# chrismile/Correrender

Hardware: AMD Instinct MI355X
Metric: Mvoxel-corr/s (higher is better)
Workload: dtype f32; 1 GPU; pearson correlation field, 256x256x256 grid x 64 ensemble members (synthetic box ensemble), one moving reference point per step; members=64, measure=pearson, resident=members and result in HBM

## Files before the change

### correrender_amd/csrc/api.cpp

```cpp
#include "../../include/corrfield.h"

#include <hip/hip_runtime.h>

#include <cstdarg>
#include <cstdlib>
#include <cstdio>
#include <cmath>
#include <cstring>
#include <functional>
#include <immintrin.h>
#include <sys/mman.h>

#include <algorithm>
#include <atomic>
#include <chrono>
#include <limits>
#include <memory>
#include <string>
#include <thread>
#include <vector>

#include "crf_context.h"
#include "crf_host_copy.h"
#include "crf_internal.h"
// ... 312 lines not shown
    if (int(current.ptrs.size()) != c->cs)
        return fail(c, CRF_ERR_STATE, "no member volumes uploaded or bound");
    return CRF_OK;
}

crf::Event take_event(crf_context* c) {
    crf::Event e;
    if (!c->ev_free.empty()) {
        e = std::move(c->ev_free.back());
        c->ev_free.pop_back();
    } else {
        (void)e.create();
    }
    return e;
}

hipStream_t stream_of(crf_context* c, void* stream) { return stream ? static_cast<hipStream_t>(stream) : c->stream; }

int launch_status(crf_context* c, hipError_t e) {
    if (e == hipSuccess) return CRF_OK;
    return fail(c, CRF_ERR_DEVICE, fmt("kernel launch failed: %s", hipGetErrorString(e)));
}

struct TimedLaunch {
    crf_context* c;
    crf::Event e0, e1;
    crf::LaunchInfo info;
    explicit TimedLaunch(crf_context* ctx, bool timed = true) : c(ctx) {
        if (c->profiling && timed) {
            e0 = take_event(c);
            e1 = take_event(c);
        }
    }
    int finish(hipError_t e) {
        c->last_kernel = info.kernel_name ? info.kernel_name : "";
        if (e0 && e1) c->ev_pending.emplace_back(std::move(e0), std::move(e1));
        return launch_status(c, e);
    }
};

int check_params(crf_context* c, const crf_params* p, int member_limit, const char* who = nullptr) {
    if (!p) return fail(c, CRF_ERR_ARGUMENT, "null argument");
    if (p->measure < CRF_PEARSON || p->measure > CRF_KMI_CC)
        return fail(c, CRF_ERR_ARGUMENT, fmt("unknown measure %d", p->measure));
    for (int v : p->reserved)
        if (v != 0) return fail(c, CRF_ERR_ARGUMENT, "crf_params.reserved must be zero");
    if (member_limit > 0 && c->cs > member_limit)
        return fail(c, CRF_ERR_UNSUPPORTED,
                    who ? fmt("%s at most %d members", who, member_limit)
                        : fmt("measure %d supports at most %d members (got %d)", p->measure, member_limit, c->cs));
    if ((p->measure == CRF_MI_BINNED || p->measure == CRF_BINNED_MI_CC) && (p->num_bins < 1 || p->num_bins > 255))
        return fail(c, CRF_ERR_ARGUMENT, fmt("num_bins %d outside [1,255]", p->num_bins));
    if ((p->measure == CRF_MI_KRASKOV || p->measure == CRF_KMI_CC) && p->k < 1)
        return fail(c, CRF_ERR_ARGUMENT, fmt("k=%d must be at least 1", p->k));
    return CRF_OK;
}

int check_slots(crf_context* c, int first, int count, bool one = false) {
    if (count >= 0 && first >= 0 && first + count <= CRF_PREPARED_SLOTS) return CRF_OK;
    return fail(c, CRF_ERR_ARGUMENT,
                one ? fmt("slot %d outside [0,%d)", first, CRF_PREPARED_SLOTS)
                    : fmt("slots [%d, %d) outside [0, %d)", first, first + count, CRF_PREPARED_SLOTS));
}

size_t launch_voxels(const crf_context* c) { return c->pipeline_voxels ? c->pipeline_voxels : c->view.num_voxels; }

int ensure_workspace(crf_context* c, size_t need) {
    for (int set = 0; set < c->pipeline_sets; set++) {
        crf_scratch& sc = c->grid.scratch[set];
// ... 363 lines not shown
                break;
            }
            e = crf::launch_mi_kraskov(c->view.members, c->cs, c->view.num_voxels, ref, ka, c->grid.tables.get(), prep, out, s,
                                       e0, e1, info);
            break;
        }
    }
    const int rc = launch.finish(e);
    if (e == hipErrorNotSupported)
        return fail(c, CRF_ERR_UNSUPPORTED, fmt("measure %d is not implemented by this build", p->measure));
    return rc;
}

int compute_impl(crf_context* c, const crf_params* p, const void* device_reference_values, void* device_out,
                 void* stream, unsigned phase, int slot, const crf::RefOverride* ov = nullptr) {
    if (!c || !c->windowed || !p || (p->flags & CRF_FLAG_SYMMETRIC))
        return compute_impl_one(c, p, device_reference_values, device_out, stream, phase, slot, ov);
    if (int r = ensure_wide(c, stream_of(c, stream))) return r;
    if (phase & 1u)
        if (int r = compute_impl_one(c, p, device_reference_values, nullptr, stream, 1u, slot, ov)) return r;
    if (!(phase & 2u)) return CRF_OK;
    if (!device_out) return fail(c, CRF_ERR_ARGUMENT, "null argument");
    return for_each_window(c, static_cast<float*>(device_out), [&](float* o) {
        return compute_impl_one(c, p, nullptr, o, stream, 2u, slot, nullptr);
    });
}

int apply_abs(crf_context* c, const crf_params* p, void* device_out, void* stream) {
    if (p->flags & CRF_FLAG_ABSOLUTE_VALUE)
        CRF_HIP(c, crf::launch_abs(static_cast<float*>(device_out), c->view.num_voxels, stream_of(c, stream)));
    return CRF_OK;
}

int ensure_host_ranges(crf_context* c, bool native) {
    crf_grid_state& g = c->grid;
    if (g.host_chunks > 0 && g.chunk_native == native) return CRF_OK;
    g.host_chunks = 0;
    const size_t n = c->alloc_voxels;
    const std::vector<size_t> first = crf::host_range_partition(n, env_int_or("CRF_HOST_CHUNKS", 0),
                                                                crf::parse_shares(getenv("CRF_HOST_SHARES")), kMaxHostChunks);
    const int ranges = int(first.size()) - 1;
    std::vector<const void*> table(size_t(ranges) * size_t(c->cs));
    const crf_member_set& set = native ? g.narrow : g.members;
    const size_t element = crf::member_format_bytes(set.format);
    for (int j = 0; j < ranges; j++)
        for (int m = 0; m < c->cs; m++)
            table[size_t(j) * size_t(c->cs) + size_t(m)] =
                static_cast<const char*>(set.ptrs[size_t(m)]) + first[size_t(j)] * element;
    CRF_HIP(c, g.chunk_tables.reserve(table.size()));
    CRF_HIP(c, hipMemcpy(g.chunk_tables.get(), table.data(), table.size() * sizeof(void*), hipMemcpyHostToDevice));
    CRF_HIP(c, c->copy_stream.create());
    for (int j = 0; j < ranges; j++) CRF_HIP(c, c->chunk_done[j].create(hipEventDisableTiming));
    for (int j = 0; j < ranges; j++) CRF_HIP(c, c->chunk_copied[j].create(hipEventDisableTiming));
    CRF_HIP(c, c->prep_done.create(hipEventDisableTiming));
    for (int j = 0; j <= ranges; j++) g.chunk_first[j] = first[size_t(j)];
    g.host_chunks = ranges;
    g.chunk_native = native;
    return CRF_OK;
}

template <class Launch>
int run_windowed(crf_context* c, void* device_out, void* stream, bool native, Launch&& launch) {
    if (int r = bind_device(c)) return r;
    hipStream_t s = stream_of(c, stream);
    if (!native)
        if (int r = ensure_wide(c, s)) return r;
// ... 410 lines not shown
                       void* stream) {
    if (p && p->prepared_slot != 0) {
        if (p->prepared_slot < 0 || p->prepared_slot > CRF_PREPARED_SLOTS)
            return fail(c, CRF_ERR_ARGUMENT, fmt("prepared_slot %d outside [0,%d]", p->prepared_slot, CRF_PREPARED_SLOTS));
        if (c && !c->prep_slots) return fail(c, CRF_ERR_STATE, "prepared_slot given but crf_prepare_device was never called");
        if (int r = compute_impl(c, p, nullptr, device_out, stream, 2u, p->prepared_slot - 1)) return r;
    } else {
        if (int r = compute_impl(c, p, device_reference_values, device_out, stream, 3u, -1)) return r;
    }
    return apply_abs(c, p, device_out, stream);
}

int crf_prepare_device(crf_context* c, const crf_params* p, const void* device_reference_values, int slot, void* stream) {
    return crf::prepare_device_ex(c, p, device_reference_values, slot, stream, nullptr);
}

int crf_prepare_rows_device(crf_context* c, const crf_params* p, const void* device_rows, int first_slot, int count,
                            void* stream) {
    if (!c || !p || !device_rows) return fail(c, CRF_ERR_ARGUMENT, "null argument");
    if (int r = check_slots(c, first_slot, count)) return r;
    crf_params local = *p;
    local.reference_values = nullptr;
    local.prepared_slot = 0;
    const float* rows = static_cast<const float*>(device_rows);
    for (int i = 0; i < count; i++)
        if (int r = crf_prepare_device(c, &local, rows + size_t(i) * size_t(c->cs), first_slot + i, stream)) return r;
    return CRF_OK;
}

int crf_compute_prepared_device(crf_context* c, const crf_params* p, int first_slot, int count, void* const* device_outs,
                                void* stream) {
    if (!c || !p || !device_outs) return fail(c, CRF_ERR_ARGUMENT, "null argument");
    if (int r = check_slots(c, first_slot, count)) return r;
    crf_params local = *p;
    for (int i = 0; i < count; i++) {
        local.prepared_slot = first_slot + i + 1;
        if (int r = crf_compute_device(c, &local, nullptr, device_outs[i], stream)) return r;
    }
    return CRF_OK;
}

int crf_compute(crf_context* c, const crf_params* p, float* host_out) {
    return crf::compute_to_host(c, p, nullptr, host_out, nullptr);
}

int crf_compute_requests_device(crf_context* c, const crf_params* p, const void* device_requests, size_t num_requests,
                                void* device_out, void* stream) {
    if (int r = check_ready(c)) return r;
    if (int r = check_params(c, p, crf::kMaxGenericMembers, "pair requests support")) return r;
    if (num_requests && (!device_requests || !device_out)) return fail(c, CRF_ERR_ARGUMENT, "null argument");
    if (c->windowed)
        return fail(c, CRF_ERR_UNSUPPORTED, "pair requests address voxels with 32-bit byte offsets: member volumes of 4 GiB or more are not supported in request mode");
    if (int r = bind_device(c)) return r;
    hipStream_t s = stream_of(c, stream);
    if (int r = ensure_wide(c, s)) return r;
    crf::TwoVectorJob job = two_vector_job(c, p);
    if (p->flags & CRF_FLAG_QUERY_FROM_SECONDARY) {
        if (!c->grid.has_secondary())
            return fail(c, CRF_ERR_STATE, "CRF_FLAG_QUERY_FROM_SECONDARY needs secondary members (crf_upload_secondary_members)");
        if (int r = ensure_secondary_wide(c, s)) return r;
        job.members_y = c->view.secondary;
    }
    job.requests = static_cast<const uint32_t*>(device_requests);
    job.num_items = num_requests;
    job.use_abs = (p->flags & CRF_FLAG_ABSOLUTE_VALUE) ? 1 : 0;
    job.out = static_cast<float*>(device_out);
// ... 292 lines not shown
    if (k < 1 || cs < 1) return std::numeric_limits<double>::quiet_NaN();
    return psi_int(cs) - psi_int(k);
}

size_t crf_tiled_element_count(int xs, int ys, int zs) {
    if (xs <= 0 || ys <= 0 || zs <= 0) return 0;
    return size_t((xs + 7) / 8) * size_t((ys + 7) / 8) * size_t((zs + 3) / 4) * 256;
}

int crf_tile_field_device(crf_context* c, const void* device_linear, void* device_tiled, void* stream) {
    if (!c) return CRF_ERR_ARGUMENT;
    if (c->cs <= 0) return fail(c, CRF_ERR_STATE, "crf_set_grid has not been called");
    if (c->windowed) return fail(c, CRF_ERR_UNSUPPORTED, "re-tiling a field of 4 GiB or more is not supported");
    if (!device_linear || !device_tiled) return fail(c, CRF_ERR_ARGUMENT, "null argument");
    if (int r = bind_device(c)) return r;
    hipStream_t s = stream_of(c, stream);
    hipError_t e = crf::launch_tile_field(static_cast<const float*>(device_linear), static_cast<float*>(device_tiled),
                                          c->xs, c->ys, c->zs, s);
    return launch_status(c, e);
}

int crf_set_profiling(crf_context* c, int enabled) {
    if (!c) return CRF_ERR_ARGUMENT;
    c->profiling = enabled != 0;
    return CRF_OK;
}

int crf_take_kernel_time(crf_context* c, double* out_ms_sum, int* out_launches) {
    if (!c || !out_ms_sum || !out_launches) return fail(c, CRF_ERR_ARGUMENT, "null argument");
    if (int r = bind_device(c)) return r;
    double sum = 0.0;
    int n = 0;
    for (auto& p : c->ev_pending) {
        CRF_HIP(c, hipEventSynchronize(p.second));
        float ms = 0.f;
        CRF_HIP(c, hipEventElapsedTime(&ms, p.first, p.second));
        sum += double(ms);
        n++;
        c->ev_free.push_back(std::move(p.first));
        c->ev_free.push_back(std::move(p.second));
    }
    c->ev_pending.clear();
    *out_ms_sum = sum;
    *out_launches = n;
    return CRF_OK;
}

const char* crf_last_kernel_name(const crf_context* c) { return c ? c->last_kernel.c_str() : ""; }

int crf_set_member_layout(crf_context* c, int mode) {
    if (!c) return CRF_ERR_ARGUMENT;
    if (mode != CRF_MEMBER_LAYOUT_AUTO && mode != CRF_MEMBER_LAYOUT_RAW && mode != CRF_MEMBER_LAYOUT_PACKED)
        return fail(c, CRF_ERR_ARGUMENT, fmt("unknown member layout %d", mode));
    if (mode == c->member_layout) return CRF_OK;
    if (int r = bind_device(c)) return r;
    CRF_HIP(c, hipDeviceSynchronize());
    drop_packed(c);
    c->member_layout = mode;
    return CRF_OK;
}

int crf_last_member_layout(const crf_context* c) { return c ? c->last_layout : CRF_MEMBER_LAYOUT_RAW; }

int crf_members_changed(crf_context* c) {
    if (!c) return CRF_ERR_ARGUMENT;
    if (int r = bind_device(c)) return r;
    CRF_HIP(c, hipDeviceSynchronize());
    primary_members_changed(c);
    secondary_members_changed(c);
    return CRF_OK;
}

int crf_synth_box_member(crf_context* c, void* device_out, int xs, int ys, int zs_local, int z_begin, int zs_global,
// ... 13 lines not shown
```

### correrender_amd/csrc/crf_context.h

```cpp
#pragma once
#include <hip/hip_runtime.h>

#include <atomic>
#include <memory>
#include <string>
#include <utility>
#include <vector>

#include "../../include/corrfield.h"
#include "crf_host_copy.h"
#include "crf_internal.h"
#include "crf_owned.h"
#include "crf_pool.h"
#include "crf_windows.h"

struct crf_scratch {
    crf::DeviceBuffer<uint32_t> todo;
    crf::DeviceBuffer<unsigned char> workspace;
};

struct crf_member_set {
    crf::DeviceBuffer<unsigned char> owned;
    std::vector<const void*> ptrs;
    crf::DeviceBuffer<const void*> table;
// ... 40 lines not shown
struct crf_launch_view {
    const float* const* members = nullptr;
    const float* const* secondary = nullptr;
    const void* const* narrow = nullptr;
    size_t num_voxels = 0;
    int max_vpt = 1;
    int scratch_set = 0;
    const void* const* secondary_narrow = nullptr;
};

struct crf_context {
    int device = -1;
    crf::Stream stream;
    std::string err;
    int xs = 0, ys = 0, zs = 0, cs = 0;
    size_t alloc_voxels = 0;
    bool windowed = false;
    size_t window_voxels = crf::kDefaultWindowVoxels;
    crf_grid_state grid;
    crf_launch_view view;
    int last_format = CRF_MEMBER_F32;
    int member_layout = CRF_MEMBER_LAYOUT_AUTO;
    int last_layout = CRF_MEMBER_LAYOUT_RAW;
    crf::DeviceBuffer<float> prep;
    crf::DeviceBuffer<float> prep_slots;
    crf::DeviceBuffer<uint32_t> minmax;
    crf::DeviceBuffer<uint32_t> pack_fallbacks;
    crf::DeviceBuffer<crf_request> requests;
    crf::DeviceBuffer<float> request_out;
    int pipeline_sets = 1;
    size_t pipeline_voxels = 0;
    bool profiling = false;
    std::vector<crf::Event> ev_free;
    std::vector<std::pair<crf::Event, crf::Event>> ev_pending;
    std::string last_kernel;
    std::atomic<int> chunk_ready[kMaxHostChunks] = {};
    crf::Stream stream2;
    crf::Stream copy_stream;
    crf::Event prep_done;
    crf::Event chunk_done[kMaxHostChunks];
    crf::Event chunk_copied[kMaxHostChunks];
    std::unique_ptr<crf::SpinPool> copy_pool;
    int copy_threads = 0;
    int copy_threads_cap = 0;
};


namespace crf {
inline hipError_t spin_on_event(hipEvent_t e) {
    const auto t0 = std::chrono::steady_clock::now();
    for (unsigned i = 1;; i++) {
        const hipError_t q = hipEventQuery(e);
        if (q != hipErrorNotReady) return q;
        if ((i & 1023u) == 0u && std::chrono::duration<double>(std::chrono::steady_clock::now() - t0).count() > 0.05)
            return hipEventSynchronize(e);
        _mm_pause();
    }
}
struct RefOverride {
    const float* const* table = nullptr;
    size_t voxel = 0;
};
int compute_to_host(crf_context* c, const crf_params* p, const void* device_reference_values, float* host_out,
                    const RefOverride* ref_override);
int compute_device_ex(crf_context* c, const crf_params* p, const void* device_reference_values, void* device_out,
                      void* stream, const RefOverride* ref_override);
int prepare_device_ex(crf_context* c, const crf_params* p, const void* device_reference_values, int slot, void* stream,
// ... 6 lines not shown
```

### correrender_amd/csrc/crf_internal.h

```cpp
#pragma once
#include <hip/hip_runtime.h>
#include <cstddef>
#include <cstdint>

#include "../../include/corrfield.h"
#include "symmetric_narrow_route.h"
#include "two_vector_route.h"

namespace crf {

constexpr int kMaxRegisterMembers = 384;
constexpr size_t kPrepBytes = 160 * 1024;
constexpr int kMaxGenericMembers = 2048;
constexpr size_t kBinnedSxOffset = kPrepBytes - 16;

struct RefSource {
    const float* values;
    size_t voxel;
    unsigned phase = 3;
    const float* const* table = nullptr;
    bool prepare() const { return (phase & 1u) != 0; }
    bool run() const { return (phase & 2u) != 0; }
};

// ... 39 lines not shown
}
__host__ __device__ inline uint32_t pack_lo16(uint32_t bits) { return bits & 0xFFFFu; }
__host__ __device__ inline uint32_t pack_byte(uint32_t bits) { return ((bits >> 24) & 0x80u) | ((bits >> 16) & 0x7Fu); }
__host__ __device__ inline uint32_t pack_code(uint32_t bits, uint32_t base) {
    const uint32_t e = (bits >> 23) & 0xFFu;
    return e == 0u ? 0u : e - base + 1u;
}
__host__ __device__ inline uint32_t perm_bytes(uint32_t hi, uint32_t lo, uint32_t sel) {
#if defined(__HIP_DEVICE_COMPILE__)
    return __builtin_amdgcn_perm(hi, lo, sel);
#else
    const uint64_t d = (uint64_t(hi) << 32) | lo;
    uint32_t r = 0;
    for (int i = 0; i < 4; i++) r |= uint32_t((d >> (8 * ((sel >> (8 * i)) & 7u))) & 0xFFu) << (8 * i);
    return r;
#endif
}
__host__ __device__ inline uint32_t unpack_bits(uint32_t lo_word, int h, uint32_t byte_word, int b, uint32_t code_word,
                                                int n, uint32_t base) {
    const uint32_t sel = uint32_t(2 * h) | uint32_t(2 * h + 1) << 8 | uint32_t(4 + b) << 16 | uint32_t(4 + b) << 24;
    const uint32_t w = perm_bytes(byte_word, lo_word, sel);
    const uint32_t code = (code_word >> (4 * n)) & 0xFu;
    const uint32_t e = code != 0u ? (code + base - 1u) << 23 : 0u;
    return (w & 0x807FFFFFu) | e;
}

struct PackedMembers {
    const unsigned char* header = nullptr;
    const unsigned char* body = nullptr;
};
hipError_t launch_pearson(const float* const* d_members, int cs, size_t num_voxels, int max_vpt, const RefSource& ref,
                          float* d_prep, float* d_out, hipStream_t s, hipEvent_t ev_begin, hipEvent_t ev_end,
                          LaunchInfo* info, const PackedMembers& packed = PackedMembers{});
hipError_t launch_pack_members(const float* const* d_members, int cs, size_t num_voxels, unsigned char* header,
                               unsigned char* body, uint32_t* d_fallbacks, hipStream_t s);
constexpr int kNarrowMaxMembers = 128;
constexpr size_t kNarrowMaxBytes = size_t(0xFFFF0000u);
constexpr size_t member_format_bytes(int format) {
    return format == CRF_MEMBER_U8 ? 1 : format == CRF_MEMBER_F32 ? 4 : 2;
}
hipError_t launch_pearson_narrow(const void* const* d_narrow, int format, int cs, size_t num_voxels, bool out_vector,
                                 const RefSource& ref, float* d_prep, float* d_out, hipStream_t s, hipEvent_t ev_begin,
                                 hipEvent_t ev_end, LaunchInfo* info);
hipError_t launch_pearson_symmetric_narrow(const void* const* d_narrow_x, const void* const* d_narrow_y, int format, int cs,
                                           size_t num_voxels, bool out_vector, float* d_out, hipStream_t s,
                                           hipEvent_t ev_begin, hipEvent_t ev_end, LaunchInfo* info);
hipError_t launch_widen_members(const void* const* d_narrow, int format, int cs, size_t num_voxels, float* d_block,
                                size_t stride, hipStream_t s);
hipError_t launch_gather_reference_narrow(const void* const* d_narrow, int format, int cs, size_t voxel, float* d_out,
                                          hipStream_t s);
hipError_t launch_gather_reference_rows_narrow(const void* const* d_narrow, int format, int cs, const GatherRows& rows,
                                               int num_rows, float* d_out, hipStream_t s);
hipError_t launch_minmax_narrow(const void* const* d_narrow, int format, int cs, size_t num_voxels, uint32_t* d_keys ,
                                hipStream_t s);
hipError_t launch_fill(float* d_out, size_t n, float value, hipStream_t s);
hipError_t launch_abs(float* d_out, size_t n, hipStream_t s);

hipError_t launch_spearman(const float* const* d_members, int cs, size_t num_voxels, const RefSource& ref,
                           float* d_prep, uint32_t* d_todo, float* d_out, hipStream_t s, hipEvent_t ev_begin,
                           hipEvent_t ev_end, LaunchInfo* info);
hipError_t launch_kendall(const float* const* d_members, int cs, size_t num_voxels, const RefSource& ref,
                          float* d_prep, uint32_t* d_todo, float* d_out, hipStream_t s, hipEvent_t ev_begin,
                          hipEvent_t ev_end, LaunchInfo* info);
constexpr int pad_pow2(int cs) { return cs <= 8 ? 8 : cs <= 16 ? 16 : cs <= 32 ? 32 : cs <= 64 ? 64 : 128; }

hipError_t launch_kendall_narrow(const void* const* d_narrow, int format, int cs, size_t num_voxels, const RefSource& ref,
// ... 159 lines not shown
```

### correrender_amd/csrc/kernels_pearson.hip

```cpp
#include "crf_device.h"
#include "crf_internal.h"
#include "crf_two_vector_device.h"

namespace crf {

constexpr int kPrepZeroFilled = 1280;

__global__ __launch_bounds__(256) void pearson_prep_kernel(RefSource src, const float* const* __restrict__ members,
                                                           int cs, float* __restrict__ prep) {
    extern __shared__ float x[];
    __shared__ float sh[2];
    for (int e = threadIdx.x; e < cs; e += blockDim.x) x[e] = load_ref(src, members, e);
    __syncthreads();
    const float n = float(cs);
    const float invN = 1.0f / n;
    const float invNm1 = 1.0f / (n - 1.0f);
    if (threadIdx.x == 0) {
        float meanX = 0.0f;
        for (int e = 0; e < cs; e++) meanX += invN * x[e];
        float varX = 0.0f;
        for (int e = 0; e < cs; e++) {
            const float d = x[e] - meanX;
            varX += invNm1 * d * d;
        }
// ... 10 lines not shown
struct VecT;
template <>
struct VecT<1> {
    using type = float;
};
template <>
struct VecT<2> {
    using type = float __attribute__((ext_vector_type(2)));
};

template <int VPT>
__device__ __forceinline__ void load_vec(const float* base, uint32_t bytes, uint32_t byte_offset, float (&dst)[VPT]) {
    const auto rsrc = make_member_rsrc(base, bytes);
    if constexpr (VPT == 1) {
        dst[0] = __uint_as_float(__builtin_amdgcn_raw_buffer_load_b32(rsrc, int(byte_offset), 0, kAuxNonTemporal));
    } else {
        const auto v = __builtin_amdgcn_raw_buffer_load_b64(rsrc, int(byte_offset), 0, kAuxNonTemporal);
        dst[0] = __uint_as_float(v[0]);
        dst[1] = __uint_as_float(v[1]);
    }
}
template <int VPT>
__device__ __forceinline__ void store_vec(float* p, const float (&src)[VPT]) {
    using V = typename VecT<VPT>::type;
    V v;
    __builtin_memcpy(&v, src, sizeof(V));
    __builtin_nontemporal_store(v, reinterpret_cast<V*>(p));
}

constexpr int pad_granule(int cs_pad) { return cs_pad <= 16 ? 8 : cs_pad <= 128 ? 16 : 32; }

typedef uint32_t u4 __attribute__((ext_vector_type(4)));

template <int CS_PAD, bool EXACT>
__device__ __forceinline__ void pearson_packed_wave(const float* const* __restrict__ members,
                                                    const float* __restrict__ prep, float* __restrict__ out,
                                                    uint32_t num_voxels, int cs, const PackedMembers& packed);

template <int CS_PAD, int VPT, bool EXACT, int MIN_WAVES, bool PACKED>
__global__ __launch_bounds__(256, MIN_WAVES) void pearson_reg_kernel(const float* const* __restrict__ members,
                                                                     const float* __restrict__ prep,
                                                                     float* __restrict__ out, uint32_t num_voxels,
                                                                     int cs, PackedMembers packed) {
    static_assert(CS_PAD <= kPrepZeroFilled, "a_e is zero-filled up to kPrepZeroFilled");
    if constexpr (PACKED) {
        static_assert(VPT == 1, "one voxel per lane: a wave is one 64-voxel tile of the packed copy");
        pearson_packed_wave<CS_PAD, EXACT>(members, prep, out, num_voxels, cs, packed);
        return;
    }
    constexpr int kFirstGuarded = EXACT ? CS_PAD : CS_PAD - pad_granule(CS_PAD);
    const auto is_member = [cs](int e) { return e < kFirstGuarded || e < cs; };
    const uint32_t v0 = (blockIdx.x * 256 + threadIdx.x) * VPT;
    const uint32_t byte_offset = v0 * 4u;
    const uint32_t bytes = num_voxels * 4u;
    float y[CS_PAD][VPT];
#pragma unroll
    for (int e = 0; e < CS_PAD; e++) {
        if (e < kFirstGuarded) {
            load_vec<VPT>(members[e], bytes, byte_offset, y[e]);
        } else if (CS_PAD >= 224) {
#pragma unroll
            for (int v = 0; v < VPT; v++) y[e][v] = 0.0f;
            if (e < cs) load_vec<VPT>(members[e], bytes, byte_offset, y[e]);
        } else {
            load_vec<VPT>(members[e < cs ? e : cs - 1], bytes, e < cs ? byte_offset : kOutOfRangeOffset, y[e]);
        }
    }
    const float n = float(cs);
    const float invN = 1.0f / n;
    const float invNm1 = 1.0f / (n - 1.0f);

    float meanY[VPT];
#pragma unroll
    for (int v = 0; v < VPT; v++) meanY[v] = 0.0f;
#pragma unroll
    for (int e = 0; e < CS_PAD; e++) {
#pragma unroll
        for (int v = 0; v < VPT; v++) meanY[v] += invN * y[e][v];
    }
    float varY[VPT];
// ... 9 lines not shown
        }
    }
    float r[VPT];
    float sdY[VPT];
#pragma unroll
    for (int v = 0; v < VPT; v++) {
        sdY[v] = sqrtf(varY[v]);
        r[v] = 0.0f;
    }
    bool guard = true;
#pragma unroll
    for (int v = 0; v < VPT; v++) guard = guard && exact_div_guard(meanY[v], sdY[v]);
    if (__all(guard)) {
        float rcp[VPT];
#pragma unroll
        for (int v = 0; v < VPT; v++) rcp[v] = 1.0f / sdY[v];
#pragma unroll
        for (int e = 0; e < CS_PAD; e++) {
            const float a = prep[e];
#pragma unroll
            for (int v = 0; v < VPT; v++) r[v] += a * exact_div(y[e][v], sdY[v], rcp[v]);
        }
    } else {
#pragma unroll
        for (int e = 0; e < CS_PAD; e++) {
            const float a = prep[e];
#pragma unroll
            for (int v = 0; v < VPT; v++) r[v] += a * (is_member(e) ? y[e][v] / sdY[v] : 0.0f);
        }
    }
    if (v0 + VPT <= num_voxels) store_vec<VPT>(out + v0, r);
}

template <int CS_PAD, bool EXACT>
__device__ __forceinline__ void pearson_packed_wave(const float* const* __restrict__ members,
                                                    const float* __restrict__ prep, float* __restrict__ out,
                                                    uint32_t num_voxels, int cs, const PackedMembers& packed) {
    static_assert(CS_PAD % 16 == 0 && CS_PAD >= 32 && CS_PAD <= kPackMaxMembers, "pack_slots() of a packed cs");
    constexpr int kLo = CS_PAD / 8, kByte = CS_PAD / 16, kCode = (CS_PAD + 31) / 32;
    constexpr uint32_t kTileBytes = 1024u * uint32_t(kLo + kByte + kCode);
    constexpr int kFirstGuarded = EXACT ? CS_PAD : CS_PAD - 16;
    const auto is_member = [cs](int e) { return e < kFirstGuarded || e < cs; };
    const uint32_t tile = blockIdx.x * 4u + uint32_t(__builtin_amdgcn_readfirstlane(int(threadIdx.x >> 6)));
    if (tile >= (num_voxels + 63u) / 64u) return;
    const uint32_t v0 = tile * 64u + (threadIdx.x & 63u);
    const uint32_t byte_offset = v0 * 4u, bytes = num_voxels * 4u;
    const uint32_t* header = reinterpret_cast<const uint32_t*>(packed.header + size_t(tile) * CS_PAD);
    const auto rsrc = __builtin_amdgcn_make_buffer_rsrc(const_cast<unsigned char*>(packed.body) + size_t(tile) * kTileBytes,
                                                        short(0), int(kTileBytes), 0x00020000);
    const int lane_bytes = int(threadIdx.x & 63u) * 16;
    u4 code[kCode], byte[kByte], lo[kLo];
#pragma unroll
    for (int r = 0; r < kCode; r++)
        code[r] = __builtin_amdgcn_raw_buffer_load_b128(rsrc, lane_bytes + 1024 * (kLo + kByte + r), 0, kAuxNonTemporal);
#pragma unroll
    for (int r = 0; r < kLo; r++) {
        if (r % 2 == 0)
            byte[r / 2] = __builtin_amdgcn_raw_buffer_load_b128(rsrc, lane_bytes + 1024 * (kLo + r / 2), 0, kAuxNonTemporal);
        lo[r] = __builtin_amdgcn_raw_buffer_load_b128(rsrc, lane_bytes + 1024 * r, 0, kAuxNonTemporal);
    }
    uint32_t hdr[CS_PAD / 4];
    uint32_t fallback = 0;
#pragma unroll
    for (int i = 0; i < CS_PAD / 4; i++) {
        hdr[i] = header[i];
        const uint32_t t = ~hdr[i];
        fallback |= (t - 0x01010101u) & ~t & 0x80808080u;
    }
    f2 y[CS_PAD / 2];
#pragma unroll
// ... 13 lines not shown
    float meanY = 0.0f;
    {
        const f2 scale = {invN, invN};
#pragma unroll
        for (int k = 0; k < CS_PAD / 2; k++) {
            const f2 t = scale * y[k];
            meanY += t[0];
            meanY += t[1];
        }
    }
    {
        const f2 mean2 = {meanY, meanY};
#pragma unroll
        for (int k = 0; k < CS_PAD / 2; k++) {
            f2 d = y[k] - mean2;
            if (2 * k >= kFirstGuarded) {
                if (!is_member(2 * k)) d[0] = 0.0f;
                if (!is_member(2 * k + 1)) d[1] = 0.0f;
            }
            y[k] = d;
        }
    }
    float varY = 0.0f;
    {
        const f2 scale = {invNm1, invNm1};
#pragma unroll
        for (int k = 0; k < CS_PAD / 2; k++) {
            const f2 t = (scale * y[k]) * y[k];
            varY += t[0];
            varY += t[1];
        }
    }
    const float sdY = sqrtf(varY);
    float r = 0.0f;
    if (__all(exact_div_guard(meanY, sdY))) {
        const float rcp = 1.0f / sdY;
        const f2 rcp2 = {rcp, rcp}, sd2 = {sdY, sdY};
#pragma unroll
        for (int k = 0; k < CS_PAD / 2; k++) {
            const f2 q0 = y[k] * rcp2;
            const f2 rem = __builtin_elementwise_fma(-q0, sd2, y[k]);
            const f2 q = __builtin_elementwise_fma(rem, rcp2, q0);
            const f2 a = {prep[2 * k], prep[2 * k + 1]};
            const f2 t = a * q;
            r += t[0];
            r += t[1];
        }
    } else {
#pragma unroll
        for (int e = 0; e < CS_PAD; e++) r += prep[e] * (is_member(e) ? y[e / 2][e % 2] / sdY : 0.0f);
    }
    if (v0 < num_voxels) store_result_nt(out + v0, r);
}

__global__ __launch_bounds__(256) void pearson_encode_kernel(const float* const* __restrict__ members,
                                                             uint32_t num_voxels, int cs,
                                                             unsigned char* __restrict__ header,
                                                             unsigned char* __restrict__ body,
                                                             uint32_t* __restrict__ fallbacks) {
    const int slots = pack_slots(cs);
    const uint32_t tile = blockIdx.x * 4u + (threadIdx.x >> 6);
    if (tile >= (num_voxels + 63u) / 64u) return;
    const int lane = int(threadIdx.x & 63u);
    const uint32_t v = tile * 64u + uint32_t(lane);
    uint32_t* lane_words = reinterpret_cast<uint32_t*>(body + size_t(tile) * pack_tile_bytes(slots) + 16 * lane);
    const int byte_run0 = pack_lo_runs(slots), code_run0 = byte_run0 + pack_byte_runs(slots);
    uint32_t lo_w = 0, byte_w = 0, code_w = 0, fell_back = 0;
#pragma unroll 1
    for (int e = 0; e < slots; e++) {
        const uint32_t bits = e < cs && v < num_voxels ? __float_as_uint(members[e][v]) : 0u;
        const uint32_t ex = (bits >> 23) & 0xFFu;
        uint32_t emin = ex != 0u ? ex : 256u, emax = ex;
#pragma unroll
        for (int o = 32; o > 0; o >>= 1) {
            emin = min(emin, uint32_t(__shfl_xor(int(emin), o)));
            emax = max(emax, uint32_t(__shfl_xor(int(emax), o)));
        }
        const uint32_t base = pack_segment_base(emin, emax, emax == 255u);
        const uint32_t b = base == kPackFallback ? 0u : bits;
        lo_w |= pack_lo16(b) << (16 * (e & 1));
        byte_w |= pack_byte(b) << (8 * (e & 3));
        code_w |= pack_code(b, base) << (4 * (e & 7));
        if ((e & 1) == 1) {
            lane_words[256 * (e / 8) + (e % 8) / 2] = lo_w;
            lo_w = 0;
// ... 768 lines not shown
__global__ void fill_kernel(float* __restrict__ out, size_t n, float value) {
    const size_t i = size_t(blockIdx.x) * blockDim.x + threadIdx.x;
    if (i < n) out[i] = value;
}

namespace {

template <int CS_PAD, int VPT>
void launch_reg(const float* const* d_members, const float* d_prep, float* d_out, size_t blocks, size_t num_voxels,
                int cs, hipStream_t s) {
    constexpr int kData = CS_PAD * VPT;
    constexpr int kMinWaves = kData <= 64 ? 4 : kData <= 128 ? 2 : kData <= 160 ? 1 : 2;
    if (cs == CS_PAD)
        hipLaunchKernelGGL((pearson_reg_kernel<CS_PAD, VPT, true, kMinWaves, false>), dim3(unsigned(blocks)), dim3(256),
                           0, s, d_members, d_prep, d_out, uint32_t(num_voxels), cs, PackedMembers{});
    else
        hipLaunchKernelGGL((pearson_reg_kernel<CS_PAD, VPT, false, kMinWaves, false>), dim3(unsigned(blocks)),
                           dim3(256), 0, s, d_members, d_prep, d_out, uint32_t(num_voxels), cs, PackedMembers{});
}

template <int CS_PAD>
void launch_reg_packed(const float* const* d_members, const float* d_prep, float* d_out, size_t num_voxels, int cs,
                       const PackedMembers& packed, hipStream_t s) {
    constexpr int kMinWaves = CS_PAD <= 64 ? 5 : 2;
    const unsigned blocks = unsigned((num_voxels + 255) / 256);
    if (cs == CS_PAD)
        hipLaunchKernelGGL((pearson_reg_kernel<CS_PAD, 1, true, kMinWaves, true>), dim3(blocks), dim3(256), 0, s,
                           d_members, d_prep, d_out, uint32_t(num_voxels), cs, packed);
    else
        hipLaunchKernelGGL((pearson_reg_kernel<CS_PAD, 1, false, kMinWaves, true>), dim3(blocks), dim3(256), 0, s,
                           d_members, d_prep, d_out, uint32_t(num_voxels), cs, packed);
}

template <int CS_PAD>
void launch_reg_vpt(int vpt, const float* const* d_members, const float* d_prep, float* d_out, size_t blocks,
                    size_t num_voxels, int cs, hipStream_t s) {
    if constexpr (CS_PAD <= 16) {
        if (vpt == 2) return launch_reg<CS_PAD, 2>(d_members, d_prep, d_out, blocks, num_voxels, cs, s);
    }
    return launch_reg<CS_PAD, 1>(d_members, d_prep, d_out, blocks, num_voxels, cs, s);
}

struct LdsKernel {
    void (*kernel)(const float* const*, const float*, float*, uint32_t, int);
    int rows;
};

template <int R, int L, int G>
LdsKernel split_kernel() {
    return {pearson_split_kernel<R, L, G, 16 * G, 2>, L};
}
template <int R, int L>
LdsKernel split_kernel(int lanes) {
    return lanes == 2 ? split_kernel<R, L, 2>() : split_kernel<R, L, 4>();
}

LdsKernel split_kernel_for(int slots, int lanes) {
    switch (slots) {
        case 160: return split_kernel<160, 0>(lanes);
        case 176: return split_kernel<176, 0>(lanes);
        case 192: return split_kernel<192, 0>(lanes);
        case 208: return split_kernel<208, 0>(lanes);
        case 224: return split_kernel<208, 16>(lanes);
        case 240: return split_kernel<216, 24>(lanes);
        case 256: return split_kernel<216, 40>(lanes);
        case 272: return split_kernel<216, 56>(lanes);
// ... 162 lines not shown
            case 48: launch_symmetric_narrow<FMT, 48>(d_x, d_y, d_out, covered, cs, out_vector, s); break;
            case 64: launch_symmetric_narrow<FMT, 64>(d_x, d_y, d_out, covered, cs, out_vector, s); break;
            case 80: launch_symmetric_narrow<FMT, 80>(d_x, d_y, d_out, covered, cs, out_vector, s); break;
            case 96: launch_symmetric_narrow<FMT, 96>(d_x, d_y, d_out, covered, cs, out_vector, s); break;
            case 112: launch_symmetric_narrow<FMT, 112>(d_x, d_y, d_out, covered, cs, out_vector, s); break;
            default: launch_symmetric_narrow<FMT, 128>(d_x, d_y, d_out, covered, cs, out_vector, s); break;
        }
    }
    if (covered < num_voxels)
        hipLaunchKernelGGL(pearson_symmetric_narrow_tail_kernel<FMT>, dim3(1), dim3(64), 0, s, d_x, d_y, d_out, covered,
                           num_voxels, cs);
}
}

hipError_t launch_pearson_symmetric_narrow(const void* const* d_narrow_x, const void* const* d_narrow_y, int format, int cs,
                                           size_t num_voxels, bool out_vector, float* d_out, hipStream_t s,
                                           hipEvent_t ev_begin, hipEvent_t ev_end, LaunchInfo* info) {
    if (!symmetric_narrow_routed(format, cs) || !d_narrow_x || !d_narrow_y || !d_out ||
        num_voxels * member_format_bytes(format) >= kNarrowMaxBytes)
        return hipErrorInvalidValue;
    if (ev_begin) (void)hipEventRecord(ev_begin, s);
    switch (format) {
        case CRF_MEMBER_U8:
            launch_symmetric_narrow_format<CRF_MEMBER_U8>(d_narrow_x, d_narrow_y, d_out, num_voxels, cs, out_vector, s);
            break;
        case CRF_MEMBER_U16:
            launch_symmetric_narrow_format<CRF_MEMBER_U16>(d_narrow_x, d_narrow_y, d_out, num_voxels, cs, out_vector, s);
            break;
        default:
            launch_symmetric_narrow_format<CRF_MEMBER_F16>(d_narrow_x, d_narrow_y, d_out, num_voxels, cs, out_vector, s);
            break;
    }
    if (info) info->kernel_name = "pearson_symmetric_narrow_kernel";
    if (ev_end) (void)hipEventRecord(ev_end, s);
    return hipGetLastError();
}

hipError_t launch_pearson(const float* const* d_members, int cs, size_t num_voxels, int max_vpt, const RefSource& ref,
                          float* d_prep, float* d_out, hipStream_t s, hipEvent_t ev_begin, hipEvent_t ev_end,
                          LaunchInfo* info, const PackedMembers& packed) {
    if (cs == 1)
        return launch_single_member(ref, d_out, num_voxels, s, ev_begin, ev_end, info);
    if (ref.prepare())
        hipLaunchKernelGGL(pearson_prep_kernel, dim3(1), dim3(256), size_t(cs) * sizeof(float), s, ref, d_members, cs,
                           d_prep);
    if (!ref.run()) return hipGetLastError();

    size_t covered = num_voxels;
    const char* name;
    hipError_t e = hipSuccess;
    if (ev_begin) (void)hipEventRecord(ev_begin, s);
    if (packed.header && cs >= kPackMinMembers && cs <= kPackMaxMembers && num_voxels > 0) {
        switch (pack_slots(cs)) {
            case 32: launch_reg_packed<32>(d_members, d_prep, d_out, num_voxels, cs, packed, s); break;
            case 48: launch_reg_packed<48>(d_members, d_prep, d_out, num_voxels, cs, packed, s); break;
            case 64: launch_reg_packed<64>(d_members, d_prep, d_out, num_voxels, cs, packed, s); break;
            case 80: launch_reg_packed<80>(d_members, d_prep, d_out, num_voxels, cs, packed, s); break;
            case 96: launch_reg_packed<96>(d_members, d_prep, d_out, num_voxels, cs, packed, s); break;
            case 112: launch_reg_packed<112>(d_members, d_prep, d_out, num_voxels, cs, packed, s); break;
            default: launch_reg_packed<128>(d_members, d_prep, d_out, num_voxels, cs, packed, s); break;
        }
        name = "pearson_reg_kernel";
    } else if (cs <= 224) {
        const int cs_pad = cs <= 8 ? 8 : cs <= 128 ? (cs + 15) / 16 * 16 : (cs + 31) / 32 * 32;
        const int vpt = cs_pad <= 16 && max_vpt >= 2 ? 2 : 1;
        covered = num_voxels / vpt * vpt;
// ... 52 lines not shown
```

Before: 28930 Mvoxel-corr/s.

## Batch several prepared Pearson reference points into one packed-member pass

Adds a batched path for crf_compute_prepared_device. For Pearson on packed f32 members, one kernel launch now evaluates 8, 4 or 2 prepared reference points. Each wave decodes and normalises a voxel's members once and accumulates dot products against R reference vectors staged in LDS, writing R output fields. This is meant to amortise the member-read and decode cost across several reference points, at the price of more registers and accumulators per thread. The profiling counter now counts evaluations per launch rather than launches.

```diff
diff --git a/correrender_amd/csrc/api.cpp b/correrender_amd/csrc/api.cpp
--- a/correrender_amd/csrc/api.cpp
+++ b/correrender_amd/csrc/api.cpp
@@ -368,9 +368,9 @@
             e1 = take_event(c);
         }
     }
-    int finish(hipError_t e) {
+    int finish(hipError_t e, int evaluations = 1) {
         c->last_kernel = info.kernel_name ? info.kernel_name : "";
-        if (e0 && e1) c->ev_pending.emplace_back(std::move(e0), std::move(e1));
+        if (e0 && e1) c->ev_pending.push_back({std::move(e0), std::move(e1), evaluations});
         return launch_status(c, e);
     }
 };
@@ -800,6 +800,53 @@
     return CRF_OK;
 }
 
+int compute_prepared_batch(crf_context* c, const crf_params* p, int first_slot, int count, void* const* device_outs,
+                           void* stream, bool* taken) {
+    *taken = false;
+    constexpr int kBatchFlags = CRF_FLAG_ABSOLUTE_VALUE | CRF_FLAG_REFERENCE_FROM_SECONDARY;
+    if (count < 2 || p->measure != CRF_PEARSON || (p->flags & ~kBatchFlags) != 0 || !c->prep_slots) return CRF_OK;
+    if (check_ready(c) != CRF_OK || c->grid.format != CRF_MEMBER_F32) return CRF_OK;
+    const size_t bytes = c->view.num_voxels * sizeof(float);
+    for (int i = 0; i < count; i++) {
+        const uintptr_t a = reinterpret_cast<uintptr_t>(device_outs[i]);
+        if (a == 0 || a % sizeof(float) != 0) return CRF_OK;
+        for (int j = 0; j < i; j++) {
+            const uintptr_t b = reinterpret_cast<uintptr_t>(device_outs[j]);
+            if (a != b && a < b + bytes && b < a + bytes) return CRF_OK;
+        }
+    }
+    if (int r = check_params(c, p, 0)) return r;
+    if (int r = bind_device(c)) return r;
+    hipStream_t s = stream_of(c, stream);
+    crf::PackedMembers packed;
+    if (int r = ensure_packed(c, s, &packed)) return r;
+    if (!packed.header) return CRF_OK;
+    *taken = true;
+    int i = 0;
+    for (int r : {8, 4, 2}) {
+        for (; count - i >= r; i += r) {
+            TimedLaunch launch(c);
+            float* outs[8];
+            for (int j = 0; j < r; j++) outs[j] = static_cast<float*>(device_outs[i + j]);
+            const float* prep = c->prep_slots.get() + size_t(first_slot + i) * (crf::kPrepBytes / sizeof(float));
+            const hipError_t e = crf::launch_pearson_prepared_batch(c->view.members, c->cs, c->view.num_voxels, prep, r, outs, s,
+                                                                    launch.e0, launch.e1, &launch.info, packed);
+            if (int rc = launch.finish(e, r)) return rc;
+        }
+    }
+    c->last_format = CRF_MEMBER_F32;
+    c->last_layout = CRF_MEMBER_LAYOUT_PACKED;
+    for (int j = 0; j < i; j++)
+        if (int r = apply_abs(c, p, device_outs[j], stream)) return r;
+    if (i < count) {
+        crf_params local = *p;
+        local.prepared_slot = first_slot + i + 1;
+        if (int r = crf_compute_device(c, &local, nullptr, device_outs[i], stream)) return r;
+        c->last_kernel = "pearson_batch_kernel";
+    }
+    return CRF_OK;
+}
+
 int ensure_host_ranges(crf_context* c, bool native) {
     crf_grid_state& g = c->grid;
     if (g.host_chunks > 0 && g.chunk_native == native) return CRF_OK;
@@ -1276,6 +1323,9 @@
                                 void* stream) {
     if (!c || !p || !device_outs) return fail(c, CRF_ERR_ARGUMENT, "null argument");
     if (int r = check_slots(c, first_slot, count)) return r;
+    bool taken = false;
+    if (int r = compute_prepared_batch(c, p, first_slot, count, device_outs, stream, &taken)) return r;
+    if (taken) return CRF_OK;
     crf_params local = *p;
     for (int i = 0; i < count; i++) {
         local.prepared_slot = first_slot + i + 1;
@@ -1634,13 +1684,13 @@
     double sum = 0.0;
     int n = 0;
     for (auto& p : c->ev_pending) {
-        CRF_HIP(c, hipEventSynchronize(p.second));
+        CRF_HIP(c, hipEventSynchronize(p.end));
         float ms = 0.f;
-        CRF_HIP(c, hipEventElapsedTime(&ms, p.first, p.second));
+        CRF_HIP(c, hipEventElapsedTime(&ms, p.begin, p.end));
         sum += double(ms);
-        n++;
-        c->ev_free.push_back(std::move(p.first));
-        c->ev_free.push_back(std::move(p.second));
+        n += p.evaluations;
+        c->ev_free.push_back(std::move(p.begin));
+        c->ev_free.push_back(std::move(p.end));
     }
     c->ev_pending.clear();
     *out_ms_sum = sum;
diff --git a/correrender_amd/csrc/crf_context.h b/correrender_amd/csrc/crf_context.h
--- a/correrender_amd/csrc/crf_context.h
+++ b/correrender_amd/csrc/crf_context.h
@@ -96,7 +96,11 @@
     size_t pipeline_voxels = 0;
     bool profiling = false;
     std::vector<crf::Event> ev_free;
-    std::vector<std::pair<crf::Event, crf::Event>> ev_pending;
+    struct TimedPair {
+        crf::Event begin, end;
+        int evaluations;
+    };
+    std::vector<TimedPair> ev_pending;
     std::string last_kernel;
     std::atomic<int> chunk_ready[kMaxHostChunks] = {};
     crf::Stream stream2;
diff --git a/correrender_amd/csrc/crf_internal.h b/correrender_amd/csrc/crf_internal.h
--- a/correrender_amd/csrc/crf_internal.h
+++ b/correrender_amd/csrc/crf_internal.h
@@ -95,6 +95,9 @@
 hipError_t launch_pearson(const float* const* d_members, int cs, size_t num_voxels, int max_vpt, const RefSource& ref,
                           float* d_prep, float* d_out, hipStream_t s, hipEvent_t ev_begin, hipEvent_t ev_end,
                           LaunchInfo* info, const PackedMembers& packed = PackedMembers{});
+hipError_t launch_pearson_prepared_batch(const float* const* d_members, int cs, size_t num_voxels, const float* d_prep,
+                                         int r, float* const* d_outs, hipStream_t s, hipEvent_t ev_begin,
+                                         hipEvent_t ev_end, LaunchInfo* info, const PackedMembers& packed);
 hipError_t launch_pack_members(const float* const* d_members, int cs, size_t num_voxels, unsigned char* header,
                                unsigned char* body, uint32_t* d_fallbacks, hipStream_t s);
 constexpr int kNarrowMaxMembers = 128;
diff --git a/correrender_amd/csrc/kernels_pearson.hip b/correrender_amd/csrc/kernels_pearson.hip
--- a/correrender_amd/csrc/kernels_pearson.hip
+++ b/correrender_amd/csrc/kernels_pearson.hip
@@ -66,9 +66,9 @@
 
 typedef uint32_t u4 __attribute__((ext_vector_type(4)));
 
-template <int CS_PAD, bool EXACT>
+template <int CS_PAD, bool EXACT, int R = 1>
 __device__ __forceinline__ void pearson_packed_wave(const float* const* __restrict__ members,
-                                                    const float* __restrict__ prep, float* __restrict__ out,
+                                                    const float* __restrict__ prep, float* const (&outs)[R],
                                                     uint32_t num_voxels, int cs, const PackedMembers& packed);
 
 template <int CS_PAD, int VPT, bool EXACT, int MIN_WAVES, bool PACKED>
@@ -79,7 +79,8 @@
     static_assert(CS_PAD <= kPrepZeroFilled, "a_e is zero-filled up to kPrepZeroFilled");
     if constexpr (PACKED) {
         static_assert(VPT == 1, "one voxel per lane: a wave is one 64-voxel tile of the packed copy");
-        pearson_packed_wave<CS_PAD, EXACT>(members, prep, out, num_voxels, cs, packed);
+        float* const outs[1] = {out};
+        pearson_packed_wave<CS_PAD, EXACT>(members, prep, outs, num_voxels, cs, packed);
         return;
     }
     constexpr int kFirstGuarded = EXACT ? CS_PAD : CS_PAD - pad_granule(CS_PAD);
@@ -155,10 +156,13 @@
     if (v0 + VPT <= num_voxels) store_vec<VPT>(out + v0, r);
 }
 
-template <int CS_PAD, bool EXACT>
+constexpr size_t kPrepFloats = kPrepBytes / sizeof(float);
+
+template <int CS_PAD, bool EXACT, int R>
 __device__ __forceinline__ void pearson_packed_wave(const float* const* __restrict__ members,
-                                                    const float* __restrict__ prep, float* __restrict__ out,
+                                                    const float* __restrict__ prep, float* const (&outs)[R],
                                                     uint32_t num_voxels, int cs, const PackedMembers& packed) {
+    static_assert(R == 1 || R % 2 == 0, "points are accumulated in pairs");
     static_assert(CS_PAD % 16 == 0 && CS_PAD >= 32 && CS_PAD <= kPackMaxMembers, "pack_slots() of a packed cs");
     constexpr int kLo = CS_PAD / 8, kByte = CS_PAD / 16, kCode = (CS_PAD + 31) / 32;
     constexpr uint32_t kTileBytes = 1024u * uint32_t(kLo + kByte + kCode);
@@ -238,6 +242,43 @@
         }
     }
     const float sdY = sqrtf(varY);
+    if constexpr (R > 1) {
+        f2 acc[R / 2];
+#pragma unroll
+        for (int p = 0; p < R / 2; p++) acc[p] = f2{0.0f, 0.0f};
+        const auto add_slot = [&](int e, float q) {
+            const f2 qq = {q, q};
+#pragma unroll
+            for (int p = 0; p < R / 2; p++) {
+                const f2 a = *reinterpret_cast<const f2*>(prep + e * R + 2 * p);
+                acc[p] = acc[p] + a * qq;
+            }
+        };
+        if (__all(exact_div_guard(meanY, sdY))) {
+            const float rcp = 1.0f / sdY;
+            const f2 rcp2 = {rcp, rcp}, sd2 = {sdY, sdY};
+#pragma unroll
+            for (int k = 0; k < CS_PAD / 2; k++) {
+                const f2 q0 = y[k] * rcp2;
+                const f2 rem = __builtin_elementwise_fma(-q0, sd2, y[k]);
+                const f2 q = __builtin_elementwise_fma(rem, rcp2, q0);
+                add_slot(2 * k, q[0]);
+                add_slot(2 * k + 1, q[1]);
+                __builtin_amdgcn_sched_barrier(0);
+            }
+        } else {
+#pragma unroll
+            for (int e = 0; e < CS_PAD; e++) {
+                add_slot(e, y[e / 2][e % 2] / (is_member(e) ? sdY : 1.0f));
+                if (e % 2 == 1) __builtin_amdgcn_sched_barrier(0);
+            }
+        }
+        if (v0 < num_voxels) {
+#pragma unroll
+            for (int j = 0; j < R; j++) store_result_nt(outs[j] + v0, acc[j / 2][j % 2]);
+        }
+        return;
+    }
     float r = 0.0f;
     if (__all(exact_div_guard(meanY, sdY))) {
         const float rcp = 1.0f / sdY;
@@ -256,7 +297,23 @@
 #pragma unroll
         for (int e = 0; e < CS_PAD; e++) r += prep[e] * (is_member(e) ? y[e / 2][e % 2] / sdY : 0.0f);
     }
-    if (v0 < num_voxels) store_result_nt(out + v0, r);
+    if (v0 < num_voxels) store_result_nt(outs[0] + v0, r);
+}
+
+template <int R>
+struct BatchOuts {
+    float* p[R];
+};
+template <int CS_PAD, bool EXACT, int MIN_WAVES, int R>
+__global__ __launch_bounds__(256, MIN_WAVES) void pearson_packed_batch_kernel(const float* const* __restrict__ members,
+                                                                              const float* __restrict__ prep,
+                                                                              BatchOuts<R> outs, uint32_t num_voxels,
+                                                                              int cs, PackedMembers packed) {
+    static_assert(CS_PAD <= kPrepZeroFilled, "a_e is zero-filled up to kPrepZeroFilled");
+    __shared__ __attribute__((aligned(16))) float a[CS_PAD * R];
+    for (int i = threadIdx.x; i < CS_PAD * R; i += 256) a[i] = prep[size_t(i % R) * kPrepFloats + i / R];
+    __syncthreads();
+    pearson_packed_wave<CS_PAD, EXACT, R>(members, a, outs.p, num_voxels, cs, packed);
 }
 
 __global__ __launch_bounds__(256) void pearson_encode_kernel(const float* const* __restrict__ members,
@@ -1091,6 +1148,29 @@
                            d_members, d_prep, d_out, uint32_t(num_voxels), cs, packed);
 }
 
+template <int CS_PAD, int R>
+void launch_reg_packed_batch(const float* const* d_members, const float* d_prep, float* const* d_outs, size_t num_voxels,
+                             int cs, const PackedMembers& packed, hipStream_t s) {
+    constexpr int kMinWaves = CS_PAD <= 64 ? 5 : 2;
+    const unsigned blocks = unsigned((num_voxels + 255) / 256);
+    BatchOuts<R> outs;
+    for (int j = 0; j < R; j++) outs.p[j] = d_outs[j];
+    if (cs == CS_PAD)
+        hipLaunchKernelGGL((pearson_packed_batch_kernel<CS_PAD, true, kMinWaves, R>), dim3(blocks), dim3(256), 0, s,
+                           d_members, d_prep, outs, uint32_t(num_voxels), cs, packed);
+    else
+        hipLaunchKernelGGL((pearson_packed_batch_kernel<CS_PAD, false, kMinWaves, R>), dim3(blocks), dim3(256), 0, s,
+                           d_members, d_prep, outs, uint32_t(num_voxels), cs, packed);
+}
+
+template <int CS_PAD>
+void launch_reg_packed_batch_r(int r, const float* const* d_members, const float* d_prep, float* const* d_outs,
+                               size_t num_voxels, int cs, const PackedMembers& packed, hipStream_t s) {
+    if (r == 8) return launch_reg_packed_batch<CS_PAD, 8>(d_members, d_prep, d_outs, num_voxels, cs, packed, s);
+    if (r == 4) return launch_reg_packed_batch<CS_PAD, 4>(d_members, d_prep, d_outs, num_voxels, cs, packed, s);
+    return launch_reg_packed_batch<CS_PAD, 2>(d_members, d_prep, d_outs, num_voxels, cs, packed, s);
+}
+
 template <int CS_PAD>
 void launch_reg_vpt(int vpt, const float* const* d_members, const float* d_prep, float* d_out, size_t blocks,
                     size_t num_voxels, int cs, hipStream_t s) {
@@ -1319,6 +1399,27 @@
             break;
     }
     if (info) info->kernel_name = "pearson_symmetric_narrow_kernel";
+    if (ev_end) (void)hipEventRecord(ev_end, s);
+    return hipGetLastError();
+}
+
+hipError_t launch_pearson_prepared_batch(const float* const* d_members, int cs, size_t num_voxels, const float* d_prep,
+                                         int r, float* const* d_outs, hipStream_t s, hipEvent_t ev_begin,
+                                         hipEvent_t ev_end, LaunchInfo* info, const PackedMembers& packed) {
+    if (!packed.header || cs < kPackMinMembers || cs > kPackMaxMembers || num_voxels == 0 ||
+        num_voxels >= (size_t(1) << 30) || (r != 2 && r != 4 && r != 8))
+        return hipErrorInvalidValue;
+    if (ev_begin) (void)hipEventRecord(ev_begin, s);
+    switch (pack_slots(cs)) {
+        case 32: launch_reg_packed_batch_r<32>(r, d_members, d_prep, d_outs, num_voxels, cs, packed, s); break;
+        case 48: launch_reg_packed_batch_r<48>(r, d_members, d_prep, d_outs, num_voxels, cs, packed, s); break;
+        case 64: launch_reg_packed_batch_r<64>(r, d_members, d_prep, d_outs, num_voxels, cs, packed, s); break;
+        case 80: launch_reg_packed_batch_r<80>(r, d_members, d_prep, d_outs, num_voxels, cs, packed, s); break;
+        case 96: launch_reg_packed_batch_r<96>(r, d_members, d_prep, d_outs, num_voxels, cs, packed, s); break;
+        case 112: launch_reg_packed_batch_r<112>(r, d_members, d_prep, d_outs, num_voxels, cs, packed, s); break;
+        default: launch_reg_packed_batch_r<128>(r, d_members, d_prep, d_outs, num_voxels, cs, packed, s); break;
+    }
+    if (info) info->kernel_name = "pearson_batch_kernel";
     if (ev_end) (void)hipEventRecord(ev_end, s);
     return hipGetLastError();
 }
```

After: 28460 Mvoxel-corr/s. 1.6% lower.
